# ZhengkunTian/OpenTransformer

Hardware: AMD Instinct MI355X
Metric: utterances/sec (80-d fbank, ~1000 frames) train fwd+bwd (higher is better)
Workload: dtype fp16; 1 GPU; AISHELL-1 transformer_baseline.yaml (+input_size 80), 12 enc / 6 dec layers, B=32/GPU x 1000 frames x 80-d fbank, 15 decoder rows, V=4234, residual_dropout 0.1; step = fwd + bwd + grad all-reduce + clip/Adam/Noam; global_batch=32, frames=1000, parallelism=dp1, hipgraph=True

## Files before the change

opentransformer_amd/csrc/api.hip:

```cpp
#include <stdarg.h>
#include <stdio.h>
#include <stdlib.h>

#include <algorithm>
#include <vector>

#include "gemm_kernel.h"
#include "wgrad256.h"

static thread_local char g_err[512] = "";

void otr_set_error(const char* fmt, ...) {
  va_list ap;
  va_start(ap, fmt);
  vsnprintf(g_err, sizeof(g_err), fmt, ap);
  va_end(ap);
}

int32_t otr_check_launch(const char* what) {
  hipError_t e = hipGetLastError();
  if (e != hipSuccess) {
    otr_set_error("%s: launch failed: %s", what, hipGetErrorString(e));
    return (int32_t)e;
  }
  return 0;
}

static __global__ void zero_f32_kernel(float* p, int64_t n) {
  for (int64_t i = (int64_t)blockIdx.x * blockDim.x + threadIdx.x; i < n; i += (int64_t)gridDim.x * blockDim.x) p[i] = 0.f;
}
void otr_zero_f32(float* p, int64_t n, hipStream_t s) {
  if (n <= 0) return;
  unsigned g = (unsigned)((n + 255) / 256 > 1024 ? 1024 : (n + 255) / 256);
  hipLaunchKernelGGL(zero_f32_kernel, dim3(g), dim3(256), 0, s, p, n);
}

int g_otr_force_tile = 0;
int g_otr_force_ksplit = 0;
int g_otr_conv2_wgrad256 = 1;
int g_otr_attn_enc96 = 1;
int g_otr_wgrad256 = -1;
int g_otr_wgrad256_grid = 0;
int g_otr_conv2_fwd_direct = 1;
int g_otr_attn_enc = 1;
int g_otr_attn_xmap = 1;
int g_otr_attn_bwd_split = 0;
int g_otr_beam_reg = 1;
int g_otr_decode_attn64 = 1;
int g_otr_dec_group = 0;
int g_otr_ffn_map = 1;
int g_otr_ffn_coh_only = 0;
int g_otr_spin_limit = 1 << 22;
int32_t* g_otr_fault = nullptr;
unsigned long long* g_otr_trace = nullptr;
extern "C" int32_t otr_debug_trace(void* buf) { g_otr_trace = (unsigned long long*)buf; return 0; }
extern "C" int32_t otr_debug_set(int32_t key, int32_t value) {
  if (key == 0) g_otr_force_tile = value;
  else if (key == 1) g_otr_force_ksplit = value;
  else if (key == 6) g_otr_wgrad256 = value;
  else if (key == 7) g_otr_wgrad256_grid = value;
  else if (key == 11) g_otr_spin_limit = value > 0 ? value : 1 << 22;
  else if (key == 12) g_otr_ffn_coh_only = value;
  else if (key == 13) g_otr_attn_bwd_split = value;
  else if (key == 15) g_otr_ffn_map = value;
  else if (key == 16) g_otr_attn_xmap = value;
  else if (key == 21) g_otr_attn_enc = value;
  else if (key == 22) g_otr_conv2_fwd_direct = value;
  else if (key == 23) g_otr_dec_group = value;
  else if (key == 24) g_otr_decode_attn64 = value;
  else if (key == 25) g_otr_beam_reg = value;
  else if (key == 29) g_otr_conv2_wgrad256 = value;
  else if (key == 30) g_otr_conv2_dgrad_wide = value;
  else if (key == 31) g_otr_conv2_wide = value;
  else if (key == 33) g_otr_attn_enc96 = value;
  else { otr_set_error("debug_set: unknown key %d", key); return -1; }
  return 0;
}

extern "C" int32_t otr_set_fault_counter(void* device_word) { g_otr_fault = (int32_t*)device_word; return 0; }

extern "C" int32_t otr_version(void) { return OTR_ABI_VERSION; }
extern "C" int32_t otr_half_type(void) { return OTR_H16; }
extern "C" const char* otr_last_error_string(void) { return g_err; }

static inline int esize(int dtype) { return dtype == OTR_F32 ? 4 : 2; }
static inline bool dtype_ok(int d) { return d == OTR_F32 || d == OTR_H16; }
static inline int kc_vec(const void* p, int64_t ld, int dtype) {
  return ((uintptr_t)p % 16 == 0) && (ld % (16 / esize(dtype)) == 0);
}
static inline int mc_vec(const void* p, int64_t ld, int dtype, int compute) {
  int pm = compute == OTR_H16 ? 4 : 2;
  return ((uintptr_t)p % (pm * esize(dtype)) == 0) && (ld % pm == 0);
}

static int32_t run_gemm(const GemmArgs& a, int compute, int ad, int bd, int cd, int amode, int bmode, void* stream) {
  if (a.M <= 0 || a.N <= 0) return 0;
  OTR_REQUIRE(a.K > 0, "gemm: K must be positive (got %d)", a.K);
  hipStream_t s = (hipStream_t)stream;
  if (compute == OTR_H16) return gemm_dispatch_bf16(a, ad, bd, cd, amode, bmode, s);
  if (compute == OTR_F32) return gemm_dispatch_f32(a, ad, bd, cd, amode, bmode, s);
  otr_set_error("gemm: bad compute type %d", compute);
  return -1;
}

static int32_t check_linear(const otr_linear_desc_t* d) {
  OTR_REQUIRE(d != nullptr, "linear: null descriptor");
  OTR_REQUIRE(d->M >= 0 && d->N >= 0 && d->K > 0, "linear: bad shape M=%d N=%d K=%d", d->M, d->N, d->K);
  OTR_REQUIRE(dtype_ok(d->x_dtype) && dtype_ok(d->w_dtype) && dtype_ok(d->y_dtype), "linear: bad dtype code");
  OTR_REQUIRE(d->ldx >= d->K && d->ldw >= d->K && d->ldy >= d->N, "linear: leading dimension smaller than row");
  return 0;
}

extern "C" int32_t otr_linear_fwd(const otr_linear_desc_t* d, const void* x, const void* w, const float* bias,
                                  void* y, void* workspace, int64_t workspace_bytes, void* stream) {
  if (int32_t e = check_linear(d)) return e;
  OTR_REQUIRE(x && w && y, "linear_fwd: null pointer");
  GemmArgs a{};
  a.A = x; a.B = w; a.C = y; a.bias = bias;
  a.M = d->M; a.N = d->N; a.K = d->K;
  a.lda = d->ldx; a.ldb = d->ldw; a.ldc = d->ldy;
  a.act = d->act; a.accumulate = d->accumulate;
  a.a_vec = kc_vec(x, d->ldx, d->x_dtype);
  a.b_vec = kc_vec(w, d->ldw, d->w_dtype);
  a.allow_split = 1; a.ws = (float*)workspace; a.ws_bytes = workspace_bytes; a.trace = g_otr_trace;
  return run_gemm(a, d->compute, d->x_dtype, d->w_dtype, d->y_dtype, MODE_KC, MODE_KC, stream);
}

extern "C" int32_t otr_linear_fwd_batched(const otr_linear_desc_t* d, const void* x, const void* w, void* y, int32_t nbatch, int64_t bsx,
                                          int64_t bsw, int64_t bsy, void* stream) {
  if (int32_t e = check_linear(d)) return e;
  OTR_REQUIRE(x && w && y, "linear_fwd_batched: null pointer");
  OTR_REQUIRE(nbatch >= 1 && nbatch <= 65535 && bsx >= 0 && bsw >= 0 && bsy > 0, "linear_fwd_batched: bad batch (n=%d)", nbatch);
  OTR_REQUIRE(d->act == OTR_ACT_NONE && !d->accumulate, "linear_fwd_batched: plain products only");
  if (nbatch == 1) return 1;
  GemmArgs a{};
  a.A = x; a.B = w; a.C = y; a.bias = nullptr;
  a.M = d->M; a.N = d->N; a.K = d->K;
  a.lda = d->ldx; a.ldb = d->ldw; a.ldc = d->ldy;
  a.act = OTR_ACT_NONE; a.accumulate = 0;
  a.a_vec = kc_vec(x, d->ldx, d->x_dtype);
  a.b_vec = kc_vec(w, d->ldw, d->w_dtype);
  a.allow_split = 0; a.ws = nullptr; a.ws_bytes = 0; a.trace = nullptr;
  a.nbatch = nbatch; a.bsa = bsx * esize(d->x_dtype); a.bsb = bsw * esize(d->w_dtype); a.bsc = bsy * esize(d->y_dtype);
  if (d->compute != OTR_H16) return 1;
  return run_gemm(a, d->compute, d->x_dtype, d->w_dtype, d->y_dtype, MODE_KC, MODE_KC, stream);
}

extern "C" int32_t otr_linear_dgrad(const otr_linear_desc_t* d, const void* dy, const void* w, void* dx,
                                    void* workspace, int64_t workspace_bytes, void* stream) {
  if (int32_t e = check_linear(d)) return e;
  OTR_REQUIRE(dy && w && dx, "linear_dgrad: null pointer");
  GemmArgs a{};
  a.A = dy; a.B = w; a.C = dx; a.bias = nullptr;
  a.M = d->M; a.N = d->K; a.K = d->N;
  a.lda = d->ldy; a.ldb = d->ldw; a.ldc = d->ldx;
  a.act = OTR_ACT_NONE; a.accumulate = d->accumulate;
  a.a_vec = kc_vec(dy, d->ldy, d->y_dtype);
// ... 273 lines not shown
```

opentransformer_amd/csrc/attention.hip:

```cpp
#include <initializer_list>

#include "common.h"

struct AttnArgs {
  const void *q, *k, *v, *o, *do_;
  void *out, *dq, *dk, *dv;
  const uint8_t* key_mask;
  float* lse;
  float* delta;
  int B, H, Tq, Tk;
  int64_t q_bs, q_ts, k_bs, k_ts, v_bs, v_ts, o_bs, o_ts;
  int causal;
  float scale;
  int vec;
  int xmap;
  const float* bias;
  int bias_vec4;
  float* dbias; int dbias_h16;
  int64_t bias_bs, bias_hs, bias_rs;
  int rel_shift;
};

__device__ __forceinline__ int64_t bias_index(const AttnArgs& p, int b, int h, int i, int j) {
  return (int64_t)b * p.bias_bs + (int64_t)h * p.bias_hs + (int64_t)i * p.bias_rs + j + (p.rel_shift ? (p.Tq - 1 - i) : 0);
// ... 668 lines not shown
      if (kmask == ~0ull && !p.causal && !p.bias) {
#pragma unroll
        for (int r = 0; r < 4; ++r) ds[kt][r] = attn_exp<CT>(s[r] * sc2 - lsf) * (dp[r] - dl) * p.scale;
        continue;
      }
#pragma unroll
      for (int r = 0; r < 4; ++r) {
        const int kl = kt * 16 + lg * 4 + r, key = kb * 64 + kl;
        bool ok = q_ok && ls != NEG_INF && ((kmask >> kl) & 1) && (!p.causal || key <= qrow);
        float raw = s[r];
        if (p.bias && ok) raw += bv[kt][r];
        float pe = ok ? attn_exp<CT>(raw * sc2 - ls) : 0.f;
        ds[kt][r] = pe * (dp[r] - dl) * p.scale;
      }
    }
#pragma unroll
    for (int c = 0; c < C::NC; ++c) {
      uint4 dsf = MMA<CT>::from_tiles(&ds[c * C::TPC]);
#pragma unroll
      for (int dt = 0; dt < C::DT; ++dt) MMA<CT>::mma(acc[dt], read_tr<CT, DK>(sKt, dt * 16 + lr, c, lg), dsf);
    }
  }
  if (q_ok) {
    CT* dQ = reinterpret_cast<CT*>(p.dq) + b * p.q_bs + (int64_t)qrow * p.q_ts + h * DK;
#pragma unroll
    for (int dt = 0; dt < C::DT; ++dt) {
      if (!row_live) acc[dt] = f32x4{0.f, 0.f, 0.f, 0.f};
      store4<CT>(dQ + dt * 16 + lg * 4, acc[dt][0], acc[dt][1], acc[dt][2], acc[dt][3], vec);
    }
  }
}
template <class CT, int DK, bool PIPE> __global__ __launch_bounds__(256) void attn_bwd_dq_kernel(AttnArgs p) {
  __shared__ __attribute__((aligned(16))) unsigned char smem[BwdSmem<CT, DK>::DQ];
  attn_bwd_dq_body<CT, DK, PIPE>(p, (int)blockIdx.x, (int)blockIdx.y, (int)blockIdx.z, smem);
}
template <class CT, int DK, int NW> __global__ __launch_bounds__(64 * NW, 2) void attn_bwd_kernel(AttnArgs p, int nqb) {
  __shared__ __attribute__((aligned(16))) unsigned char smem[BwdSmem<CT, DK>::BOTH];
  int bx, h, b;
  if (!attn_block(p, nqb + (p.Tk + 16 * NW - 1) / (16 * NW), bx, h, b)) return;
  if (bx < nqb) attn_bwd_dq_body<CT, DK, true, NW>(p, bx, h, b, smem);
  else attn_bwd_dkdv_body<CT, DK, true, true, NW>(p, bx - nqb, h, b, smem);
}

static int32_t fill_args(const otr_attn_desc_t* d, AttnArgs& a) {
  OTR_REQUIRE(d != nullptr, "attention: null descriptor");
  OTR_REQUIRE(d->B > 0 && d->H > 0 && d->Tq > 0 && d->Tk > 0, "attention: bad shape B=%d H=%d Tq=%d Tk=%d", d->B, d->H,
              d->Tq, d->Tk);
  OTR_REQUIRE(d->dtype == OTR_F32 || d->dtype == OTR_H16, "attention: bad dtype %d", d->dtype);
  OTR_REQUIRE(d->dk == 16 || d->dk == 32 || d->dk == 64 || d->dk == 96 || d->dk == 128,
              "attention: head dim %d not built (16/32/64/96/128)", d->dk);
  a.B = d->B; a.H = d->H; a.Tq = d->Tq; a.Tk = d->Tk;
  a.q_bs = d->q_bs; a.q_ts = d->q_ts; a.k_bs = d->k_bs; a.k_ts = d->k_ts;
  a.v_bs = d->v_bs; a.v_ts = d->v_ts; a.o_bs = d->o_bs; a.o_ts = d->o_ts;
  a.causal = d->causal; a.scale = d->scale;
  return 0;
}
static dim3 attn_grid(AttnArgs& a, const otr_attn_desc_t* d, int nx) {
  a.xmap = g_otr_attn_xmap;
  return a.xmap ? dim3((unsigned)(8 * nx * ((d->H * d->B + 7) / 8))) : dim3((unsigned)nx, d->H, d->B);
}
static int vec_ok(const otr_attn_desc_t* d, std::initializer_list<const void*> ptrs) {
  int ce = d->dtype == OTR_F32 ? 4 : 8;
  int64_t strides[] = {d->q_bs, d->q_ts, d->k_bs, d->k_ts, d->v_bs, d->v_ts, d->o_bs, d->o_ts};
  for (int64_t s : strides)
    if (s % ce) return 0;
  if (d->dk % ce) return 0;
  for (const void* p : ptrs)
    if (p && ((uintptr_t)p % 16)) return 0;
  return 1;
}

#define DK_SWITCH_P(CTYPE, KERNEL, GRID, PIPE)                                                            \
  switch (d->dk) {                                                                                        \
    case 16: hipLaunchKernelGGL((KERNEL<CTYPE, 16, PIPE>), GRID, dim3(256), 0, s, a); break;              \
    case 32: hipLaunchKernelGGL((KERNEL<CTYPE, 32, PIPE>), GRID, dim3(256), 0, s, a); break;              \
    case 64: hipLaunchKernelGGL((KERNEL<CTYPE, 64, PIPE>), GRID, dim3(256), 0, s, a); break;              \
    case 96: hipLaunchKernelGGL((KERNEL<CTYPE, 96, PIPE>), GRID, dim3(256), 0, s, a); break;              \
    default: hipLaunchKernelGGL((KERNEL<CTYPE, 128, PIPE>), GRID, dim3(256), 0, s, a); break;             \
  }
#define DK_SWITCH(CTYPE, KERNEL, GRID)                    \
  if (a.vec) { DK_SWITCH_P(CTYPE, KERNEL, GRID, true) }   \
  else { DK_SWITCH_P(CTYPE, KERNEL, GRID, false) }

extern "C" int32_t otr_attention_fwd(const otr_attn_desc_t* d, const void* q, const void* k, const void* v,
                                     const uint8_t* key_mask, void* o, float* lse, void* stream) {
  AttnArgs a{};
  if (int32_t e = fill_args(d, a)) return e;
  OTR_REQUIRE(q && k && v && o && lse, "attention_fwd: null pointer");
  a.q = q; a.k = k; a.v = v; a.out = o; a.lse = lse; a.key_mask = key_mask;
  a.vec = vec_ok(d, {q, k, v, o});
  hipStream_t s = (hipStream_t)stream;
  if (a.vec && d->dtype == OTR_H16 && d->dk == 64) {
    hipLaunchKernelGGL((attn_fwd_kernel<bf16_t, 64, true, 8>), attn_grid(a, d, (d->Tq + 127) / 128), dim3(512), 0, s, a);
    return otr_check_launch("attention_fwd");
  }
  dim3 grid = attn_grid(a, d, (d->Tq + 63) / 64);
  if (d->dtype == OTR_H16) { DK_SWITCH(bf16_t, attn_fwd_kernel, grid) } else { DK_SWITCH(float, attn_fwd_kernel, grid) }
  return otr_check_launch("attention_fwd");
}

static void set_bias(AttnArgs& a, const float* bias, float* dbias, int64_t bs, int64_t hs, int64_t rs, int rel_shift) {
  a.bias = bias; a.dbias = dbias; a.bias_bs = bs; a.bias_hs = hs; a.bias_rs = rs; a.rel_shift = rel_shift;
  a.bias_vec4 = 0;
  if (rel_shift && bs >= 0 && hs >= 0 && rs >= 0) {
    const int64_t T = a.Tq, k64 = ((int64_t)a.Tk + 63) / 64 * 64, H = a.H;
    int64_t extent = 0, reach = 0;
    for (int64_t h : {(int64_t)0, H - 1})
      for (int64_t i : {(int64_t)0, T - 1}) {
        extent = std::max(extent, h * hs + i * rs + 2 * T - 1);
        reach = std::max(reach, h * hs + i * rs + (k64 - 1) + (T - 1 - i) + 1);
      }
    a.bias_vec4 = reach <= extent;
  }
}

extern "C" int32_t otr_attention_bias_fwd(const otr_attn_desc_t* d, const void* q, const void* k, const void* v,
                                          const uint8_t* key_mask, const float* bias, int64_t bias_bs, int64_t bias_hs,
                                          int64_t bias_rs, int32_t rel_shift, void* o, float* lse, void* stream) {
  AttnArgs a{};
  if (int32_t e = fill_args(d, a)) return e;
  OTR_REQUIRE(q && k && v && o && lse && bias, "attention_bias_fwd: null pointer");
  OTR_REQUIRE(!rel_shift || d->Tq == d->Tk, "attention_bias_fwd: rel_shift needs Tq == Tk");
  a.q = q; a.k = k; a.v = v; a.out = o; a.lse = lse; a.key_mask = key_mask;
  a.vec = vec_ok(d, {q, k, v, o});
  set_bias(a, bias, nullptr, bias_bs, bias_hs, bias_rs, rel_shift);
  hipStream_t s = (hipStream_t)stream;
  if (a.vec && d->dtype == OTR_H16 && d->dk == 64) {
    hipLaunchKernelGGL((attn_fwd_kernel<bf16_t, 64, true, 8>), attn_grid(a, d, (d->Tq + 127) / 128), dim3(512), 0, s, a);
    return otr_check_launch("attention_bias_fwd");
  }
  dim3 grid = attn_grid(a, d, (d->Tq + 63) / 64);
  if (d->dtype == OTR_H16) { DK_SWITCH(bf16_t, attn_fwd_kernel, grid) } else { DK_SWITCH(float, attn_fwd_kernel, grid) }
  return otr_check_launch("attention_bias_fwd");
}

static int32_t attention_bwd_impl(const otr_attn_desc_t* d, AttnArgs& a, void* stream);

extern "C" int32_t otr_attention_bias_bwd(const otr_attn_desc_t* d, const void* q, const void* k, const void* v,
                                          const uint8_t* key_mask, const float* bias, void* dbias, int32_t dbias_dtype, int64_t bias_bs,
                                          int64_t bias_hs, int64_t bias_rs, int32_t rel_shift, const void* o,
                                          const void* do_, const float* lse, float* delta, void* dq, void* dk, void* dv,
                                          void* stream) {
  AttnArgs a{};
  if (int32_t e = fill_args(d, a)) return e;
  OTR_REQUIRE(q && k && v && o && do_ && lse && delta && dq && dk && dv && bias, "attention_bias_bwd: null pointer");
  OTR_REQUIRE(dbias_dtype == OTR_F32 || dbias_dtype == OTR_H16, "attention_bias_bwd: bad dbias dtype %d", dbias_dtype);
  a.dbias_h16 = dbias_dtype == OTR_H16;
  a.q = q; a.k = k; a.v = v; a.o = o; a.do_ = do_; a.lse = const_cast<float*>(lse); a.delta = delta;
  a.dq = dq; a.dk = dk; a.dv = dv; a.key_mask = key_mask;
  a.vec = vec_ok(d, {q, k, v, o, do_, dq, dk, dv});
  set_bias(a, bias, reinterpret_cast<float*>(dbias), bias_bs, bias_hs, bias_rs, rel_shift);
  return attention_bwd_impl(d, a, stream);
}

extern "C" int32_t otr_attention_bwd(const otr_attn_desc_t* d, const void* q, const void* k, const void* v,
                                     const uint8_t* key_mask, const void* o, const void* do_, const float* lse,
                                     float* delta, void* dq, void* dk, void* dv, void* stream) {
  AttnArgs a{};
  if (int32_t e = fill_args(d, a)) return e;
  OTR_REQUIRE(q && k && v && o && do_ && lse && delta && dq && dk && dv, "attention_bwd: null pointer");
  a.q = q; a.k = k; a.v = v; a.o = o; a.do_ = do_; a.lse = const_cast<float*>(lse); a.delta = delta;
  a.dq = dq; a.dk = dk; a.dv = dv; a.key_mask = key_mask;
  a.vec = vec_ok(d, {q, k, v, o, do_, dq, dk, dv});
  return attention_bwd_impl(d, a, stream);
}

bool encattn_bwd_takes(int dtype_is_h16, int dk, int Tq, int Tk, int causal, int has_bias, int vec);
bool encattn96_bwd_takes(int dtype_is_h16, int dk, int Tq, int Tk, int causal, int has_bias, int rel_shift, int bias_vec4, int has_dbias, int vec);
int32_t encattn96_bwd_launch(const void* q, const void* k, const void* v, const void* o, const void* do_, const float* lse, const uint8_t* key_mask,
                             const float* bias, void* dbias, int dbias_h16, int64_t bias_bs, int64_t bias_hs, int64_t bias_rs, void* dq, void* dk,
                             void* dv, int B, int H, int T, int64_t q_bs, int64_t q_ts, int64_t k_bs, int64_t k_ts, int64_t v_bs, int64_t v_ts,
                             int64_t o_bs, int64_t o_ts, float scale, hipStream_t stream);
int32_t encattn_bwd_launch(const void* q, const void* k, const void* v, const void* o, const void* do_, const float* lse, const uint8_t* key_mask,
                           void* dq, void* dk, void* dv, int B, int H, int T, int64_t q_bs, int64_t q_ts, int64_t k_bs, int64_t k_ts, int64_t v_bs,
// ... 55 lines not shown
```

opentransformer_amd/csrc/common.h:

```cpp
#pragma once
#include <hip/hip_runtime.h>
#include <stdint.h>

#include "../../include/otrans_hip.h"

#ifdef OTR_HALF_FP16
typedef _Float16 otr_hreal;
#define OTR_H16 OTR_F16
#else
typedef __bf16 otr_hreal;
#define OTR_H16 OTR_BF16
#endif
typedef __attribute__((ext_vector_type(8))) otr_hreal bf16x8;
typedef __attribute__((ext_vector_type(2))) otr_hreal bf16x2;
typedef __attribute__((ext_vector_type(4))) float f32x4;
typedef __attribute__((ext_vector_type(2))) float f32x2;
typedef uint16_t bf16_t;

void otr_set_error(const char* fmt, ...);
int32_t otr_check_launch(const char* what);
void otr_zero_f32(float* p, int64_t n, hipStream_t s);
#define OTR_REQUIRE(cond, ...)          \
  do {                                  \
    if (!(cond)) {                      \
      otr_set_error(__VA_ARGS__);       \
      return -1;                        \
    }                                   \
  } while (0)

extern int g_otr_force_tile;
extern int g_otr_force_ksplit;
extern int g_otr_conv2_wgrad256;
extern int g_otr_attn_enc96;
extern int g_otr_wgrad256;
extern int g_otr_wgrad256_grid;
extern int g_otr_conv2_dgrad_wide;
extern int g_otr_conv2_wide;
extern int g_otr_conv2_fwd_direct;
extern int g_otr_attn_enc;
extern int g_otr_attn_xmap;
extern int g_otr_attn_bwd_split;
extern int g_otr_beam_reg;
extern int g_otr_decode_attn64;
extern int g_otr_dec_group;
extern int g_otr_ffn_map;
extern int g_otr_ffn_coh_only;
extern int g_otr_spin_limit;
extern int32_t* g_otr_fault;
extern unsigned long long* g_otr_trace;

typedef uint32_t otr_u32x4 __attribute__((ext_vector_type(4)));
typedef uint32_t otr_u32x2 __attribute__((ext_vector_type(2)));
#define OTR_GLOBAL __attribute__((address_space(1)))
__device__ __forceinline__ uint4 ld_global_b128(const void* p) {
  otr_u32x4 v = *(const OTR_GLOBAL otr_u32x4*)(p);
  return make_uint4(v.x, v.y, v.z, v.w);
}
__device__ __forceinline__ uint2 ld_global_b64(const void* p) {
  otr_u32x2 v = *(const OTR_GLOBAL otr_u32x2*)(p);
  return make_uint2(v.x, v.y);
}
__device__ __forceinline__ void st_global_b128(void* p, uint4 v) {
  otr_u32x4 t = {v.x, v.y, v.z, v.w};
  *(OTR_GLOBAL otr_u32x4*)(p) = t;
}

__device__ __forceinline__ void st_global_b128_nt(void* p, uint4 v) {
  otr_u32x4 t = {v.x, v.y, v.z, v.w};
#if defined(OTR_ST_WT) && OTR_ST_WT
  asm volatile("global_store_dwordx4 %0, %1, off sc0 sc1 nt\n\ts_nop 1" ::"v"(p), "v"(t) : "memory");
#else
  __builtin_nontemporal_store(t, (OTR_GLOBAL otr_u32x4*)(p));
#endif
}

#ifdef OTR_HALF_FP16
__device__ __forceinline__ float bf2f(bf16_t v) { return (float)__builtin_bit_cast(_Float16, v); }
__device__ __forceinline__ float h2f_lo(uint32_t w) { return bf2f((bf16_t)(w & 0xffffu)); }
__device__ __forceinline__ float h2f_hi(uint32_t w) { return bf2f((bf16_t)(w >> 16)); }
#else
__device__ __forceinline__ float bf2f(bf16_t v) { return __uint_as_float(((uint32_t)v) << 16); }
__device__ __forceinline__ float h2f_lo(uint32_t w) { return __uint_as_float(w << 16); }
__device__ __forceinline__ float h2f_hi(uint32_t w) { return __uint_as_float(w & 0xffff0000u); }
#endif
__device__ __forceinline__ bf16_t f2bf(float f) {
  otr_hreal h = (otr_hreal)f;
  return __builtin_bit_cast(bf16_t, h);
}
__device__ __forceinline__ uint32_t pack2bf(float lo, float hi) {
  f32x2 v = {lo, hi};
  bf16x2 h = __builtin_convertvector(v, bf16x2);
  return __builtin_bit_cast(uint32_t, h);
}

__device__ __forceinline__ float h2f(bf16_t v) { return bf2f(v); }
__device__ __forceinline__ bf16_t f2h(float f) { return f2bf(f); }
__device__ __forceinline__ uint32_t pack2h(float lo, float hi) { return pack2bf(lo, hi); }

typedef __attribute__((ext_vector_type(16))) float f32x16;
__device__ __forceinline__ void mma32(f32x16& acc, const uint4& a, const uint4& b) {
#ifdef OTR_HALF_FP16
  acc = __builtin_amdgcn_mfma_f32_32x32x16_f16(__builtin_bit_cast(bf16x8, a), __builtin_bit_cast(bf16x8, b), acc, 0, 0, 0);
#else
  acc = __builtin_amdgcn_mfma_f32_32x32x16_bf16(__builtin_bit_cast(bf16x8, a), __builtin_bit_cast(bf16x8, b), acc, 0, 0, 0);
#endif
}

#ifdef OTR_HALF_FP16
#define OTR_MFMA32_OP "v_mfma_f32_32x32x16_f16"
#else
#define OTR_MFMA32_OP "v_mfma_f32_32x32x16_bf16"
#endif
__device__ __forceinline__ void mma32_agpr_b(f32x16& acc, const otr_u32x4& a, const otr_u32x4& b_acc) {
  asm volatile("s_nop 1\n\t" OTR_MFMA32_OP " %0, %1, %2, %0" : "+v"(acc) : "v"(a), "a"(b_acc));
}
__device__ __forceinline__ void mma32_agpr_a(f32x16& acc, const otr_u32x4& a_acc, const otr_u32x4& b) {
  asm volatile("s_nop 1\n\t" OTR_MFMA32_OP " %0, %1, %2, %0" : "+v"(acc) : "a"(a_acc), "v"(b));
}

typedef __attribute__((address_space(3))) unsigned char lds_byte;

template <bool NT = false> __device__ __forceinline__ void lds_dma(const void* src, uint32_t lds_dst) {
  uint32_t keep;
  if constexpr (NT)
    asm volatile("s_mov_b32 %0, m0\n\ts_mov_b32 m0, %2\n\ts_nop 0\n\tglobal_load_lds_dwordx4 %1, off nt\n\ts_mov_b32 m0, %0"
                 : "=&s"(keep) : "v"(src), "s"(lds_dst) : "memory");
  else
    asm volatile("s_mov_b32 %0, m0\n\ts_mov_b32 m0, %2\n\ts_nop 0\n\tglobal_load_lds_dwordx4 %1, off\n\ts_mov_b32 m0, %0"
                 : "=&s"(keep) : "v"(src), "s"(lds_dst) : "memory");
}
__device__ __forceinline__ void lds_dma_sbase(const void* uniform_src, uint32_t lane_off, uint32_t lds_dst) {
  uint32_t keep;
  asm volatile("s_mov_b32 %0, m0\n\ts_mov_b32 m0, %3\n\ts_nop 0\n\tglobal_load_lds_dwordx4 %1, %2\n\ts_mov_b32 m0, %0"
               : "=&s"(keep) : "v"(lane_off), "s"(uniform_src), "s"(lds_dst) : "memory");
}
template <int N> __device__ __forceinline__ void wait_vm() { asm volatile("s_waitcnt vmcnt(%0)" ::"n"(N) : "memory"); }
__device__ __forceinline__ void wait_lds() { asm volatile("s_waitcnt lgkmcnt(0)" ::: "memory"); }

constexpr int OTR_STAMP_BASE = 16384;
constexpr int OTR_KID_DECLAYER = 0, OTR_KID_ENCATTN = 6, OTR_KID_CONV2FWD = 9;
#define OTR_STAMP(TRACE, KID, UNIT, K, LIVE)                                                                    \
  do {                                                                                                          \
    if ((TRACE) && threadIdx.x == 0 && (LIVE))                                                                  \
      (TRACE)[OTR_STAMP_BASE + ((KID) * 256 + (UNIT)) * 16 + (K)] = __builtin_amdgcn_s_memtime();               \
  } while (0)

template <class T> struct ElemIO;
template <> struct ElemIO<float> {
  static __device__ __forceinline__ float ld(const float* p) { return *p; }
  static __device__ __forceinline__ void st(float* p, float v) { *p = v; }
};
template <> struct ElemIO<bf16_t> {
  static __device__ __forceinline__ float ld(const bf16_t* p) { return bf2f(*p); }
  static __device__ __forceinline__ void st(bf16_t* p, float v) { *p = f2bf(v); }
};

template <class CT> struct MMA;
template <> struct MMA<bf16_t> {
  static constexpr int CE = 8;
  static constexpr int KSTEP = 32;
  static constexpr int TPC = 2;
  static __device__ __forceinline__ void mma(f32x4& acc, const uint4& a, const uint4& b) {
#ifdef OTR_HALF_FP16
    acc = __builtin_amdgcn_mfma_f32_16x16x32_f16(__builtin_bit_cast(bf16x8, a), __builtin_bit_cast(bf16x8, b), acc, 0, 0, 0);
#else
    acc = __builtin_amdgcn_mfma_f32_16x16x32_bf16(__builtin_bit_cast(bf16x8, a), __builtin_bit_cast(bf16x8, b), acc, 0, 0, 0);
#endif
  }
  static __device__ __forceinline__ uint4 pack(const float* f) {
    uint4 r;
    r.x = pack2bf(f[0], f[1]);
    r.y = pack2bf(f[2], f[3]);
    r.z = pack2bf(f[4], f[5]);
    r.w = pack2bf(f[6], f[7]);
    return r;
  }
  static __device__ __forceinline__ uint4 from_tiles(const f32x4* t) {
    uint4 r;
    r.x = pack2bf(t[0][0], t[0][1]);
    r.y = pack2bf(t[0][2], t[0][3]);
    r.z = pack2bf(t[1][0], t[1][1]);
    r.w = pack2bf(t[1][2], t[1][3]);
    return r;
  }
};
template <> struct MMA<float> {
  static constexpr int CE = 4;
  static constexpr int KSTEP = 16;
  static constexpr int TPC = 1;
  static __device__ __forceinline__ void mma(f32x4& acc, const uint4& a, const uint4& b) {
    acc = __builtin_amdgcn_mfma_f32_16x16x4f32(__uint_as_float(a.x), __uint_as_float(b.x), acc, 0, 0, 0);
    acc = __builtin_amdgcn_mfma_f32_16x16x4f32(__uint_as_float(a.y), __uint_as_float(b.y), acc, 0, 0, 0);
    acc = __builtin_amdgcn_mfma_f32_16x16x4f32(__uint_as_float(a.z), __uint_as_float(b.z), acc, 0, 0, 0);
    acc = __builtin_amdgcn_mfma_f32_16x16x4f32(__uint_as_float(a.w), __uint_as_float(b.w), acc, 0, 0, 0);
  }
  static __device__ __forceinline__ uint4 pack(const float* f) {
    return make_uint4(__float_as_uint(f[0]), __float_as_uint(f[1]), __float_as_uint(f[2]), __float_as_uint(f[3]));
  }
  static __device__ __forceinline__ uint4 from_tiles(const f32x4* t) {
    return make_uint4(__float_as_uint(t[0][0]), __float_as_uint(t[0][1]), __float_as_uint(t[0][2]),
                      __float_as_uint(t[0][3]));
  }
};

template <class ST, int N>
__device__ __forceinline__ void load_row(const ST* p, int nvalid, bool vec, float* out) {
  if (vec && nvalid >= N) {
    if constexpr (sizeof(ST) == 4) {
#pragma unroll
      for (int i = 0; i < N; i += 4) {
        float4 v = *reinterpret_cast<const float4*>(p + i);
        out[i] = v.x; out[i + 1] = v.y; out[i + 2] = v.z; out[i + 3] = v.w;
      }
    } else {
      if constexpr (N == 8) {
        uint4 v = *reinterpret_cast<const uint4*>(p);
        out[0] = h2f_lo(v.x); out[1] = h2f_hi(v.x);
        out[2] = h2f_lo(v.y); out[3] = h2f_hi(v.y);
        out[4] = h2f_lo(v.z); out[5] = h2f_hi(v.z);
        out[6] = h2f_lo(v.w); out[7] = h2f_hi(v.w);
      } else {
        static_assert(N == 4, "bf16 rows are read 4 or 8 at a time");
        uint2 v = *reinterpret_cast<const uint2*>(p);
// ... 77 lines not shown
```

opentransformer_amd/csrc/encattn.hip:

```cpp
#include "tile32.h"

namespace {

constexpr int EA_T = 256;
constexpr int EA_TMAX = 512;
constexpr int EA_DK = 64;
constexpr int EA_HS = EA_DK * 2 + 16;
constexpr int EA_TS = EA_T * 2 + 8;
constexpr int EA_RM = EA_T * EA_HS;
constexpr int EA_TR = EA_DK * EA_TS;
constexpr float EA_LOG2E = 1.4426950408889634f;

struct EaArgs {
  unsigned long long* trace;
  const uint16_t *q, *k, *v, *o, *do_;
  uint16_t *dq, *dk, *dv;
  const uint8_t* key_mask;
  const float* lse;
  int B, H, T;
  int64_t q_bs, q_ts, k_bs, k_ts, v_bs, v_ts, o_bs, o_ts;
  float scale;
};


// ... 186 lines not shown
    float l0 = lse[min(tid, T - 1)];
    const uint8_t kmb = km ? km[ownc] : (uint8_t)1;
#pragma unroll
    for (int c = 0; c < 4; ++c) {
      gq[c] = ea_issue(Q, p.q_ts, T, tid, c);
      gdo[c] = ea_issue(dO, p.o_ts, T, tid, c);
      go[c] = ea_issue(O, p.o_ts, T, tid, c);
    }
    __builtin_amdgcn_sched_barrier(0);
    OTR_STAMP(p.trace, OTR_KID_ENCATTN + orient, g, 1, g < 256);
    const bool keyok = own < T && kmb;
    f32x16 dk[2], dv[2];
    tile_zero(dk[0]); tile_zero(dk[1]); tile_zero(dv[0]); tile_zero(dv[1]);
    auto tile = [&](int it) {
      const unsigned char* qr = qrm + it * 32 * EA_HS;
      const unsigned char* dr = dorm + it * 32 * EA_HS;
      f32x16 st, dp;
      tile_zero(st); tile_zero(dp);
#pragma unroll
      for (int ks = 0; ks < 4; ++ks) { mma32(st, frag_rm(qr, EA_HS, m, hi, ks), kf[ks]); mma32(dp, frag_rm(dr, EA_HS, m, hi, ks), vf[ks]); }
      float pv[16], dsv[16];
#pragma unroll
      for (int q = 0; q < 4; ++q) {
        const float4 nl = *reinterpret_cast<const float4*>(nls + it * 32 + 8 * q + 4 * hi);
        const float4 de = *reinterpret_cast<const float4*>(dels + it * 32 + 8 * q + 4 * hi);
        const float nl4[4] = {nl.x, nl.y, nl.z, nl.w}, de4[4] = {de.x, de.y, de.z, de.w};
#pragma unroll
        for (int e = 0; e < 4; ++e) {
          const int r = 4 * q + e;
          pv[r] = __builtin_amdgcn_exp2f(__builtin_fmaf(st[r], sc2, nl4[e]));
          dsv[r] = pv[r] * (dp[r] - de4[e]);
        }
      }
#pragma unroll
      for (int k2 = 0; k2 < 2; ++k2) {
        const uint4 pb = frag_pack8(pv + 8 * k2), sb = frag_pack8(dsv + 8 * k2);
#pragma unroll
        for (int ct = 0; ct < 2; ++ct) {
          mma32(dv[ct], frag_tr(dot, EA_TS, 32 * ct + m, it * 32, hi, k2), pb);
          mma32(dk[ct], frag_tr(qt, EA_TS, 32 * ct + m, it * 32, hi, k2), sb);
        }
      }
    };
    for (int s0 = 0; s0 < (MULTI ? T : 1); s0 += EA_T) {
      const int Ts = MULTI ? min(EA_T, T - s0) : T, nt = (Ts + 31) >> 5;
      if (MULTI && s0 > 0) {
        __syncthreads();
        l0 = lse[min(s0 + tid, T - 1)];
#pragma unroll
        for (int c = 0; c < 4; ++c) {
          gq[c] = ea_issue(Q + (int64_t)s0 * p.q_ts, p.q_ts, Ts, tid, c);
          gdo[c] = ea_issue(dO + (int64_t)s0 * p.o_ts, p.o_ts, Ts, tid, c);
          go[c] = ea_issue(O + (int64_t)s0 * p.o_ts, p.o_ts, Ts, tid, c);
        }
      }
      if (tid < EA_T) nls[tid] = (tid < Ts && l0 != -__builtin_huge_valf()) ? -l0 * EA_LOG2E : -__builtin_huge_valf();
#pragma unroll
      for (int c = 0; c < 4; ++c) {
        if (2 * c >= nt) break;
        ea_stage_rm<false>(qrm, gq[c], gq[c], nullptr, Ts, tid, c);
        ea_stage_rm<true>(dorm, gdo[c], go[c], dels, Ts, tid, c);
        __syncthreads();
        if (tid < 256) ea_transpose(qt, qrm, c, tid, 0, 4);
        else ea_transpose(dot, dorm, c, tid - 256, 0, 4);
        __syncthreads();
        if (c == 0) OTR_STAMP(p.trace, OTR_KID_ENCATTN + orient, g, 2, g < 256);
        if (wave_live) {
          tile(2 * c);
          if (2 * c + 1 < nt) tile(2 * c + 1);
        }
      }
    }
    OTR_STAMP(p.trace, OTR_KID_ENCATTN + orient, g, 3, g < 256);
    __syncthreads();
    OTR_STAMP(p.trace, OTR_KID_ENCATTN + orient, g, 4, g < 256);
    if (wave_live) {
      ea_store_rows(dk, p.scale, keyok, qrm + 32 * wid * EA_HS, p.dk + (int64_t)b * p.k_bs + h * EA_DK, p.k_ts, o0 + 32 * wid, T, lane);
      ea_store_rows(dv, 1.f, keyok, dorm + 32 * wid * EA_HS, p.dv + (int64_t)b * p.v_bs + h * EA_DK, p.v_ts, o0 + 32 * wid, T, lane);
    }
    OTR_STAMP(p.trace, OTR_KID_ENCATTN + orient, g, 5, g < 256);
  }
}

}

bool encattn_bwd_takes(int dtype_is_h16, int dk, int Tq, int Tk, int causal, int has_bias, int vec) {
  return dtype_is_h16 && dk == EA_DK && Tq == Tk && Tq >= 1 && Tq <= EA_TMAX && !causal && !has_bias && vec;
}

int32_t encattn_bwd_launch(const void* q, const void* k, const void* v, const void* o, const void* do_, const float* lse, const uint8_t* key_mask,
                           void* dq, void* dk, void* dv, int B, int H, int T, int64_t q_bs, int64_t q_ts, int64_t k_bs, int64_t k_ts, int64_t v_bs,
                           int64_t v_ts, int64_t o_bs, int64_t o_ts, float scale, hipStream_t stream) {
  EaArgs p{};
  p.trace = g_otr_trace;
  p.q = (const uint16_t*)q; p.k = (const uint16_t*)k; p.v = (const uint16_t*)v; p.o = (const uint16_t*)o; p.do_ = (const uint16_t*)do_;
  p.dq = (uint16_t*)dq; p.dk = (uint16_t*)dk; p.dv = (uint16_t*)dv; p.key_mask = key_mask; p.lse = lse;
  p.B = B; p.H = H; p.T = T; p.q_bs = q_bs; p.q_ts = q_ts; p.k_bs = k_bs; p.k_ts = k_ts; p.v_bs = v_bs; p.v_ts = v_ts; p.o_bs = o_bs; p.o_ts = o_ts;
  p.scale = scale;
  if (T <= EA_T) {
    const unsigned grid = 8u * 2u * (unsigned)((H * B + 7) / 8);
    hipLaunchKernelGGL(encattn_bwd_kernel<false>, dim3(grid), dim3(512), 0, stream, p);
  } else {
    const unsigned nob = (unsigned)((T + EA_T - 1) / EA_T);
    const unsigned grid = 8u * 2u * nob * (unsigned)((H * B + 7) / 8);
    hipLaunchKernelGGL(encattn_bwd_kernel<true>, dim3(grid), dim3(512), 0, stream, p);
  }
  return otr_check_launch("encattn_bwd");
}
```

Before: 7992 utterances/s.

## Add specialized encoder self-attention forward kernel staging full K/V in LDS

Adds a dedicated forward attention kernel for encoder self-attention (dk=64, non-causal, 256<T<=512). Each workgroup owns 256 query rows of one head and stages K and V in shared memory in two 256-key superchunks, with V transposed. It computes all score tiles of a superchunk in registers and then does a single online-softmax rescale per superchunk. Grid mapping is XCD-aware and mirrors the existing backward kernel. The goal is to cut repeated K/V global reads and per-tile rescale overhead versus the generic flash kernel, at the cost of high register and LDS use (one block per CU).

```diff
diff --git a/opentransformer_amd/csrc/api.hip b/opentransformer_amd/csrc/api.hip
--- a/opentransformer_amd/csrc/api.hip
+++ b/opentransformer_amd/csrc/api.hip
@@ -43,6 +43,7 @@
 int g_otr_wgrad256_grid = 0;
 int g_otr_conv2_fwd_direct = 1;
 int g_otr_attn_enc = 1;
+int g_otr_attn_enc_fwd = 1;
 int g_otr_attn_xmap = 1;
 int g_otr_attn_bwd_split = 0;
 int g_otr_beam_reg = 1;
@@ -73,6 +74,7 @@
   else if (key == 30) g_otr_conv2_dgrad_wide = value;
   else if (key == 31) g_otr_conv2_wide = value;
   else if (key == 33) g_otr_attn_enc96 = value;
+  else if (key == 34) g_otr_attn_enc_fwd = value;
   else { otr_set_error("debug_set: unknown key %d", key); return -1; }
   return 0;
 }
diff --git a/opentransformer_amd/csrc/attention.hip b/opentransformer_amd/csrc/attention.hip
--- a/opentransformer_amd/csrc/attention.hip
+++ b/opentransformer_amd/csrc/attention.hip
@@ -774,6 +774,11 @@
   if (a.vec) { DK_SWITCH_P(CTYPE, KERNEL, GRID, true) }   \
   else { DK_SWITCH_P(CTYPE, KERNEL, GRID, false) }
 
+bool encattn_fwd_takes(int dtype_is_h16, int dk, int Tq, int Tk, int causal, int has_bias, int vec);
+int32_t encattn_fwd_launch(const void* q, const void* k, const void* v, const uint8_t* key_mask, void* o, float* lse, int B, int H, int T,
+                           int64_t q_bs, int64_t q_ts, int64_t k_bs, int64_t k_ts, int64_t v_bs, int64_t v_ts, int64_t o_bs, int64_t o_ts,
+                           float scale, hipStream_t stream);
+
 extern "C" int32_t otr_attention_fwd(const otr_attn_desc_t* d, const void* q, const void* k, const void* v,
                                      const uint8_t* key_mask, void* o, float* lse, void* stream) {
   AttnArgs a{};
@@ -782,6 +787,8 @@
   a.q = q; a.k = k; a.v = v; a.out = o; a.lse = lse; a.key_mask = key_mask;
   a.vec = vec_ok(d, {q, k, v, o});
   hipStream_t s = (hipStream_t)stream;
+  if (g_otr_attn_enc_fwd && encattn_fwd_takes(d->dtype == OTR_H16, d->dk, d->Tq, d->Tk, a.causal, 0, a.vec))
+    return encattn_fwd_launch(q, k, v, key_mask, o, lse, d->B, d->H, d->Tq, a.q_bs, a.q_ts, a.k_bs, a.k_ts, a.v_bs, a.v_ts, a.o_bs, a.o_ts, a.scale, s);
   if (a.vec && d->dtype == OTR_H16 && d->dk == 64) {
     hipLaunchKernelGGL((attn_fwd_kernel<bf16_t, 64, true, 8>), attn_grid(a, d, (d->Tq + 127) / 128), dim3(512), 0, s, a);
     return otr_check_launch("attention_fwd");
diff --git a/opentransformer_amd/csrc/common.h b/opentransformer_amd/csrc/common.h
--- a/opentransformer_amd/csrc/common.h
+++ b/opentransformer_amd/csrc/common.h
@@ -38,6 +38,7 @@
 extern int g_otr_conv2_wide;
 extern int g_otr_conv2_fwd_direct;
 extern int g_otr_attn_enc;
+extern int g_otr_attn_enc_fwd;
 extern int g_otr_attn_xmap;
 extern int g_otr_attn_bwd_split;
 extern int g_otr_beam_reg;
@@ -138,7 +139,7 @@
 __device__ __forceinline__ void wait_lds() { asm volatile("s_waitcnt lgkmcnt(0)" ::: "memory"); }
 
 constexpr int OTR_STAMP_BASE = 16384;
-constexpr int OTR_KID_DECLAYER = 0, OTR_KID_ENCATTN = 6, OTR_KID_CONV2FWD = 9;
+constexpr int OTR_KID_DECLAYER = 0, OTR_KID_ENCATTN = 6, OTR_KID_ENCATTN_FWD = 8, OTR_KID_CONV2FWD = 9;
 #define OTR_STAMP(TRACE, KID, UNIT, K, LIVE)                                                                    \
   do {                                                                                                          \
     if ((TRACE) && threadIdx.x == 0 && (LIVE))                                                                  \
diff --git a/opentransformer_amd/csrc/encattn.hip b/opentransformer_amd/csrc/encattn.hip
--- a/opentransformer_amd/csrc/encattn.hip
+++ b/opentransformer_amd/csrc/encattn.hip
@@ -292,6 +292,167 @@
   }
 }
 
+struct EaFwdArgs {
+  unsigned long long* trace;
+  const uint16_t *q, *k, *v;
+  uint16_t* o;
+  const uint8_t* key_mask;
+  float* lse;
+  int B, H, T;
+  int64_t q_bs, q_ts, k_bs, k_ts, v_bs, v_ts, o_bs, o_ts;
+  float scale;
+};
+
+constexpr int EA_FWD_SMEM = 2 * EA_RM + EA_TR + EA_T * 4;
+
+__global__ __launch_bounds__(512, 1) void encattn_fwd_kernel(EaFwdArgs p) {
+  __shared__ __attribute__((aligned(16))) unsigned char smem[EA_FWD_SMEM];
+  const int tid = threadIdx.x, lane = tid & 63, m = lane & 31, hi = lane >> 5;
+  const int wid = __builtin_amdgcn_readfirstlane(tid >> 6);
+  const int xcd = (int)blockIdx.x & 7, kk = (int)blockIdx.x >> 3;
+  const int T = p.T;
+  const int ob = kk & 1, g = (kk >> 1) * 8 + xcd;
+  if (g >= p.H * p.B) return;
+  const int h = g % p.H, b = g / p.H;
+  const int o0 = ob * EA_T;
+  const float sc2 = p.scale * EA_LOG2E;
+  const float ninf = -__builtin_huge_valf();
+  const uint16_t* Q = p.q + (int64_t)b * p.q_bs + h * EA_DK;
+  const uint16_t* K = p.k + (int64_t)b * p.k_bs + h * EA_DK;
+  const uint16_t* V = p.v + (int64_t)b * p.v_bs + h * EA_DK;
+  const uint8_t* km = p.key_mask ? p.key_mask + (int64_t)b * T : nullptr;
+  const int own = o0 + 32 * wid + m;
+  const int ownc = min(own, T - 1);
+  const bool wave_live = o0 + 32 * wid < T;
+  const bool stamp = g < 256 && ob == 0;
+  OTR_STAMP(p.trace, OTR_KID_ENCATTN_FWD, g, 0, stamp);
+
+  unsigned char* krm = smem;
+  unsigned char* vrm = smem + EA_RM;
+  unsigned char* vt = smem + 2 * EA_RM;
+  float* kbias = reinterpret_cast<float*>(smem + 2 * EA_RM + EA_TR);
+  uint4 gk[4], gv[4], qf[4];
+  ea_load_frags(qf, Q, p.q_ts, ownc, hi);
+  uint8_t kmb = km ? km[min(tid, T - 1)] : (uint8_t)1;
+#pragma unroll
+  for (int c = 0; c < 4; ++c) {
+    gk[c] = ea_issue(K, p.k_ts, EA_T, tid, c);
+    gv[c] = ea_issue(V, p.v_ts, EA_T, tid, c);
+  }
+  __builtin_amdgcn_sched_barrier(0);
+  OTR_STAMP(p.trace, OTR_KID_ENCATTN_FWD, g, 1, stamp);
+
+  f32x16 o[2];
+  tile_zero(o[0]); tile_zero(o[1]);
+  float mrun = ninf, l = 0.f;
+  auto stile = [&](f32x16& s, float& mx, int jt) {
+    tile_zero(s);
+#pragma unroll
+    for (int ks = 0; ks < 4; ++ks) mma32(s, frag_rm(krm + jt * 32 * EA_HS, EA_HS, m, hi, ks), qf[ks]);
+#pragma unroll
+    for (int q = 0; q < 4; ++q) {
+      const float4 kb = *reinterpret_cast<const float4*>(kbias + jt * 32 + 8 * q + 4 * hi);
+      const float kb4[4] = {kb.x, kb.y, kb.z, kb.w};
+#pragma unroll
+      for (int e = 0; e < 4; ++e) {
+        s[4 * q + e] = __builtin_fmaf(s[4 * q + e], sc2, kb4[e]);
+        mx = fmaxf(mx, s[4 * q + e]);
+      }
+    }
+  };
+  auto superchunk = [&](int s0, int Ts) {
+    const int nt = (Ts + 31) >> 5;
+    if (s0 > 0) {
+      __syncthreads();
+      ea_load_frags(qf, Q, p.q_ts, ownc, hi);
+      kmb = km ? km[min(s0 + tid, T - 1)] : (uint8_t)1;
+#pragma unroll
+      for (int c = 0; c < 4; ++c) {
+        gk[c] = ea_issue(K + (int64_t)s0 * p.k_ts, p.k_ts, Ts, tid, c);
+        gv[c] = ea_issue(V + (int64_t)s0 * p.v_ts, p.v_ts, Ts, tid, c);
+      }
+    }
+    if (tid < EA_T) kbias[tid] = (tid < Ts && kmb) ? 0.f : ninf;
+    float mx = ninf;
+    f32x16 st[8];
+#pragma unroll
+    for (int c = 0; c < 4; ++c) {
+      if (2 * c >= nt) break;
+      ea_stage_rm<false>(krm, gk[c], gk[c], nullptr, Ts, tid, c);
+      ea_stage_rm<false>(vrm, gv[c], gv[c], nullptr, Ts, tid, c);
+      __syncthreads();
+      ea_transpose(vt, vrm, c, tid & 255, 2 * (tid >> 8), 2);
+      if (c == 0 && s0 == 0) OTR_STAMP(p.trace, OTR_KID_ENCATTN_FWD, g, 2, stamp);
+      if (wave_live) {
+        stile(st[2 * c], mx, 2 * c);
+        if (2 * c + 1 < nt) stile(st[2 * c + 1], mx, 2 * c + 1);
+      }
+    }
+    if (s0 > 0) OTR_STAMP(p.trace, OTR_KID_ENCATTN_FWD, g, 3, stamp);
+    float msafe = 0.f;
+    if (wave_live) {
+      mx = fmaxf(mx, __shfl_xor(mx, 32));
+      const float mnew = fmaxf(mrun, mx);
+      msafe = (mnew == ninf) ? 0.f : mnew;
+      const float alpha = __builtin_amdgcn_exp2f(mrun - msafe);
+      l *= alpha;
+#pragma unroll
+      for (int ct = 0; ct < 2; ++ct)
+#pragma unroll
+        for (int r = 0; r < 16; ++r) o[ct][r] *= alpha;
+      mrun = mnew;
+    }
+    __syncthreads();
+    if (wave_live) {
+      float rs = 0.f;
+#pragma unroll
+      for (int jt = 0; jt < 8; ++jt) {
+        if (jt >= nt) break;
+        float pv[16];
+#pragma unroll
+        for (int r = 0; r < 16; ++r) {
+          pv[r] = __builtin_amdgcn_exp2f(st[jt][r] - msafe);
+          rs += pv[r];
+        }
+#pragma unroll
+        for (int k2 = 0; k2 < 2; ++k2) {
+          const uint4 pb = frag_pack8(pv + 8 * k2);
+#pragma unroll
+          for (int ct = 0; ct < 2; ++ct) mma32(o[ct], frag_tr(vt, EA_TS, 32 * ct + m, jt * 32, hi, k2), pb);
+        }
+      }
+      rs += __shfl_xor(rs, 32);
+      l += rs;
+    }
+  };
+  superchunk(0, EA_T);
+  superchunk(EA_T, T - EA_T);
+  OTR_STAMP(p.trace, OTR_KID_ENCATTN_FWD, g, 4, stamp);
+  if (wave_live) {
+    const bool alive = l > 0.f;
+    ea_store_rows(o, alive ? 1.f / l : 0.f, alive, vrm + 32 * wid * EA_HS, p.o + (int64_t)b * p.o_bs + h * EA_DK, p.o_ts, o0 + 32 * wid, T, lane);
+    if (hi == 0 && own < T) p.lse[((int64_t)b * p.H + h) * T + own] = alive ? mrun * (1.f / EA_LOG2E) + logf(l) : ninf;
+  }
+  OTR_STAMP(p.trace, OTR_KID_ENCATTN_FWD, g, 5, stamp);
+}
+
+}
+
+bool encattn_fwd_takes(int dtype_is_h16, int dk, int Tq, int Tk, int causal, int has_bias, int vec) {
+  return dtype_is_h16 && dk == EA_DK && Tq == Tk && Tq > EA_T && Tq <= EA_TMAX && !causal && !has_bias && vec;
+}
+
+int32_t encattn_fwd_launch(const void* q, const void* k, const void* v, const uint8_t* key_mask, void* o, float* lse, int B, int H, int T,
+                           int64_t q_bs, int64_t q_ts, int64_t k_bs, int64_t k_ts, int64_t v_bs, int64_t v_ts, int64_t o_bs, int64_t o_ts,
+                           float scale, hipStream_t stream) {
+  EaFwdArgs p{};
+  p.trace = g_otr_trace;
+  p.q = (const uint16_t*)q; p.k = (const uint16_t*)k; p.v = (const uint16_t*)v; p.o = (uint16_t*)o; p.key_mask = key_mask; p.lse = lse;
+  p.B = B; p.H = H; p.T = T; p.q_bs = q_bs; p.q_ts = q_ts; p.k_bs = k_bs; p.k_ts = k_ts; p.v_bs = v_bs; p.v_ts = v_ts; p.o_bs = o_bs; p.o_ts = o_ts;
+  p.scale = scale;
+  const unsigned grid = 8u * 2u * (unsigned)((H * B + 7) / 8);
+  hipLaunchKernelGGL(encattn_fwd_kernel, dim3(grid), dim3(512), 0, stream, p);
+  return otr_check_launch("encattn_fwd");
 }
 
 bool encattn_bwd_takes(int dtype_is_h16, int dk, int Tq, int Tk, int causal, int has_bias, int vec) {
```

New measurement: 7998 utterances/s, median of 4. Within noise of the previous version (+0.1%).
